# yewzijian/RegTR

Hardware: NVIDIA H100
Metric: pairs/sec on 3DMatch-size clouds (~20k pts); pose err vs ref (higher is better)
Workload: dtype f32

## Files before the change

### include/regtr_b200.h

```cpp
#ifndef REGTR_B200_H_
#define REGTR_B200_H_

#include <stddef.h>
#include <stdint.h>

#ifdef __cplusplus
extern "C" {
#endif

#define REGTR_OK 0
#define REGTR_ERR_ARG (-1)
#define REGTR_ERR_WORKSPACE (-2)
#define REGTR_ERR_UNSUPPORTED (-3)

#define REGTR_STATUS_KEY_RANGE 1u
#define REGTR_STATUS_CAPACITY 2u
#define REGTR_STATUS_GRID 4u
#define REGTR_STATUS_RANGE 8u

int regtr_version(void);
const char* regtr_build_info(void);


size_t regtr_grid_subsample_ws_bytes(int n_cap, int n_clouds);
// ... 11 lines not shown
size_t regtr_cellgrid_state_bytes(int n_cap);
int regtr_cellgrid_build(const float* xyz, const int32_t* offs, int n_clouds, int n_cap, float cell,
                         void* grid, int32_t* order, uint32_t* status,
                         void* ws, size_t ws_bytes, void* state, size_t state_bytes, void* stream);

int regtr_ball_query(const float* q, const int32_t* q_offs, const int32_t* q_order,
                     const float* s, const int32_t* s_offs, const void* s_grid,
                     int n_clouds, int nq_cap, int s_cap, int K, float radius,
                     int32_t* out_idx32, int64_t* out_idx64, void* stream);


size_t regtr_kpconv_ws_bytes(int Nq, int Ns, int Cin);
size_t regtr_kpconv_fwd_ws_bytes(int Nq, int Ns, int Cin, int Cout);
int regtr_kpconv_fwd(const float* q, const float* s, const int32_t* idx, const float* x,
                     const float* W, const float* kp, int Nq, int Ns, const int32_t* nq_dev,
                     const int32_t* ns_dev, int K, int Cin, int Cout,
                     float extent, float* out, void* ws, size_t ws_bytes, void* stream);

int regtr_kpconv_aggregate(const float* q, const float* s, const int32_t* idx, const float* x,
                           const float* kp, int Nq, int Ns, const int32_t* nq_dev, const int32_t* ns_dev,
                           int K, int Cin, float extent,
                           float* wf, uint8_t* rowflag_ws, int flags_ready, void* stream);

int regtr_max_pool(const float* x, const int32_t* idx, int Nq, int Ns, const int32_t* ns_dev, int K, int C,
                   float* out, void* stream);

size_t regtr_instnorm_ws_bytes(int n_cap, int n_clouds, int C);
size_t regtr_instnorm_counter_bytes(int n_clouds, int C);
int regtr_instnorm_act(const float* x, const int32_t* offs, int n_clouds, int n_cap, int C, float eps,
                       const float* res, float slope, float* out, uint8_t* rowflag_out,
                       void* ws, size_t ws_bytes, int32_t* counters, void* stream);

int regtr_instnorm_apply(const float* x, const int32_t* offs, int n_clouds, int n_cap, int C, const float* stats,
                         const float* res, float slope, float* out, uint8_t* rowflag_out, void* stream);


int regtr_split_tf32(const float* x, long long n, float* hi, float* lo, void* stream);

size_t regtr_gemm_ws_bytes(int M, int N, int K);
int regtr_gemm_tf32x3(const float* A, int lda, const float* B_hi, const float* B_lo, int ldb,
                      float* C, int ldc, const float* bias, const float* R, int ldr,
                      int M, int N, int K, const int32_t* m_dev, int relu,
                      void* ws, size_t ws_bytes, void* stream);

size_t regtr_instnorm_part_bytes(int M, int N);
int regtr_gemm_tf32x3_instats(const float* A, int lda, const float* B_hi, const float* B_lo, int ldb,
                              float* C, int ldc, int M, int N, int K, const int32_t* m_dev,
                              const int32_t* offs, int n_clouds, float eps, void* part, float* stats,
                              void* ws, size_t ws_bytes, void* stream);


int regtr_pos_embed_sine(const float* xyz, int n, const float* dim_t, int n_freq, int d_model,
                         float scale, float* out, void* stream);

typedef struct regtr_dropout_args {
    unsigned long long seed, step;
    int32_t pair_base;
    int32_t layer;
    int32_t site;
    uint32_t threshold;
    float scale;
    int32_t n_pairs;
} regtr_dropout_args;

int regtr_layernorm_pos(const float* x, const float* z, const float* gamma, const float* beta, const float* pos, int n,
                        const int32_t* n_dev, const int32_t* offs, int E, float eps, float* y, float* y_pos,
                        float* x_out, const regtr_dropout_args* drop, void* stream);
// ... 354 lines not shown
```

### regtr_b200/csrc/common.cuh

```cuda
#pragma once
#include <cuda_runtime.h>
#include <stdint.h>

#include "../../include/regtr_b200.h"

#define REGTR_NUM_SMS 132

#define REGTR_CHECK_LAUNCH()                                         \
    do {                                                             \
        cudaError_t e__ = cudaGetLastError();                        \
        if (e__ != cudaSuccess) return -(1000 + (int)e__);           \
    } while (0)

static inline int regtr_cdiv(long long a, long long b) { return (int)((a + b - 1) / b); }
static inline size_t regtr_align(size_t x, size_t a = 256) { return (x + a - 1) / a * a; }

__device__ __forceinline__ unsigned long long regtr_pack_key(int cloud, int x, int y, int z) {
    return ((unsigned long long)(unsigned)cloud << 48) | ((unsigned long long)(unsigned)(x + 32768) << 32) |
           ((unsigned long long)(unsigned)(y + 32768) << 16) | (unsigned long long)(unsigned)(z + 32768);
}

__device__ __forceinline__ int regtr_cell_of(float p, float cell) { return (int)floorf(__fdiv_rn(p, cell)); }

__device__ __forceinline__ int regtr_cloud_of(const int32_t* __restrict__ offs, int n_clouds, int i) {
    int lo = 0, hi = n_clouds;
    while (hi - lo > 1) {
        int mid = (lo + hi) >> 1;
        if (offs[mid] <= i) lo = mid; else hi = mid;
    }
    return lo;
}

__device__ __forceinline__ void regtr_row_col(unsigned t, unsigned w, int& row, int& col) {
    if ((w & (w - 1u)) == 0u) { const int sh = 31 - __clz((int)w); row = (int)(t >> sh); col = (int)(t & (w - 1u)); }
    else { row = (int)(t / w); col = (int)(t - (unsigned)row * w); }
}

__device__ __forceinline__ float regtr_tf32_rne(float x) {
    uint32_t u = __float_as_uint(x);
    u += 0x0FFFu + ((u >> 13) & 1u);
    return __uint_as_float(u & 0xFFFFE000u);
}

__device__ __forceinline__ float warp_sum(float v) {
#pragma unroll
    for (int o = 16; o > 0; o >>= 1) v += __shfl_xor_sync(0xffffffffu, v, o);
    return v;
}
__device__ __forceinline__ double warp_sum(double v) {
#pragma unroll
    for (int o = 16; o > 0; o >>= 1) v += __shfl_xor_sync(0xffffffffu, v, o);
    return v;
}
__device__ __forceinline__ float warp_max(float v) {
#pragma unroll
    for (int o = 16; o > 0; o >>= 1) v = fmaxf(v, __shfl_xor_sync(0xffffffffu, v, o));
    return v;
}
```

### regtr_b200/csrc/norm.cu

```cuda
#include "common.cuh"
#include "philox.cuh"

namespace {

constexpr int IN_CH = 128;
constexpr int IN_TY = 8;
constexpr int IN_CT = 128;

__device__ __forceinline__ bool chunk_of(const int32_t* __restrict__ offs, int n_clouds, int chunk, int& cloud,
                                         int& r0, int& r1, int& first, int& count) {
    int acc = 0;
    for (int c = 0; c < n_clouds; ++c) {
        const int a = offs[c], b = offs[c + 1];
        const int nc = (b - a + IN_CH - 1) / IN_CH;
        if (chunk < acc + nc) {
            cloud = c;
            r0 = a + (chunk - acc) * IN_CH;
            r1 = min(r0 + IN_CH, b);
            first = acc;
            count = nc;
            return true;
        }
        acc += nc;
    }
// ... 74 lines not shown
        }
    }
}

__global__ void __launch_bounds__(32 * IN_TY)
k_in_finalize(const int32_t* __restrict__ offs, int n_clouds, int C, float eps, const double2* __restrict__ partial,
              float2* __restrict__ stats) {
    __shared__ double2 red[IN_TY][32];
    const int cloud = blockIdx.x;
    const int c = blockIdx.y * 32 + threadIdx.x;
    int first = 0;
    for (int k = 0; k < cloud; ++k) first += (offs[k + 1] - offs[k] + IN_CH - 1) / IN_CH;
    const int n = offs[cloud + 1] - offs[cloud];
    const int nc = (n + IN_CH - 1) / IN_CH;
    double s = 0.0, ss = 0.0;
    if (c < C) {
        for (int t = threadIdx.y; t < nc; t += IN_TY) {
            const double2 p = partial[(size_t)(first + t) * C + c];
            s += p.x; ss += p.y;
        }
    }
    red[threadIdx.y][threadIdx.x] = make_double2(s, ss);
    __syncthreads();
    if (threadIdx.y == 0 && c < C) {
        for (int t = 1; t < IN_TY; ++t) { s += red[t][threadIdx.x].x; ss += red[t][threadIdx.x].y; }
        const double dn = n > 0 ? (double)n : 1.0;
        const double mean = s / dn;
        double var = ss / dn - mean * mean;
        var = var > 0.0 ? var : 0.0;
        stats[(size_t)cloud * C + c] = make_float2((float)mean, (float)(1.0 / sqrt(var + (double)eps)));
    }
}

template <bool FLAGS>
__global__ void k_in_apply(const float* x, const int32_t* __restrict__ offs, int n_clouds, int n_cap, int C,
                           const float2* __restrict__ stats, const float* res, float slope, float* out,
                           uint8_t* __restrict__ flags) {
    const int c4n = C >> 2;
    const int n_real = offs[n_clouds];
    const unsigned total = (unsigned)min(n_cap, (n_real + 127) & ~127) * (unsigned)c4n;
    const unsigned stride = gridDim.x * blockDim.x;
    for (unsigned t0 = blockIdx.x * blockDim.x; t0 < total; t0 += stride) {
        const unsigned t = t0 + threadIdx.x;
        const bool in_range = t < total;
        int r = 0, c = 0;
        if (in_range) { regtr_row_col(t, (unsigned)c4n, r, c); c *= 4; }
        const size_t o = (size_t)r * C + c;
        const bool live = in_range && r < n_real;
        float y[4] = {0.f, 0.f, 0.f, 0.f};
        if (live) {
            const float4 v = *reinterpret_cast<const float4*>(x + o);
            float4 rv = make_float4(0.f, 0.f, 0.f, 0.f);
            if (res) rv = *reinterpret_cast<const float4*>(res + o);
            const int cloud = regtr_cloud_of(offs, n_clouds, r);
            const float4 st01 = *reinterpret_cast<const float4*>(stats + (size_t)cloud * C + c);
            const float4 st23 = *reinterpret_cast<const float4*>(stats + (size_t)cloud * C + c + 2);
            y[0] = (v.x - st01.x) * st01.y + rv.x; y[1] = (v.y - st01.z) * st01.w + rv.y;
            y[2] = (v.z - st23.x) * st23.y + rv.z; y[3] = (v.w - st23.z) * st23.w + rv.w;
            if (slope >= 0.f) {
#pragma unroll
                for (int j = 0; j < 4; ++j) y[j] = y[j] > 0.f ? y[j] : y[j] * slope;
            }
        }
        if (in_range) *reinterpret_cast<float4*>(out + o) = make_float4(y[0], y[1], y[2], y[3]);
        if (FLAGS) {
            double acc = ((double)y[0] + (double)y[1]) + ((double)y[2] + (double)y[3]);
            for (int d = 1; d < c4n; d <<= 1) acc += __shfl_xor_sync(0xffffffffu, acc, d);
            if (in_range && (threadIdx.x & (c4n - 1)) == 0) flags[r] = live && acc > 0.0;
        }
    }
}

template <int PER, bool DROP = false>
__global__ void k_layernorm_pos(const float* __restrict__ x, const float* __restrict__ gamma,
                                const float* __restrict__ beta, const float* __restrict__ pos, int n,
                                const int32_t* __restrict__ n_dev, int E, float eps, float* __restrict__ y,
                                float* __restrict__ y_pos, const float* __restrict__ z = nullptr,
                                float* __restrict__ x_out = nullptr, DropKey drop = DropKey{}) {
    const int row = (blockIdx.x * blockDim.x + threadIdx.x) >> 5, lane = threadIdx.x & 31;
    if (!DROP && n_dev) n = min(n, *n_dev);
    if (row >= n) return;
    const float* xr = x + (size_t)row * E;
    const int per = E / 32;
    float v[PER], gm[PER], bt[PER], ps[PER];
#pragma unroll
    for (int j = 0; j < PER; ++j)
        if (j < per) {
            const int c = j * 32 + lane;
            v[j] = xr[c]; gm[j] = __ldg(gamma + c); bt[j] = __ldg(beta + c);
            ps[j] = (y_pos && pos) ? pos[(size_t)row * E + c] : 0.f;
        }
    if constexpr (DROP) {
        const int cl = regtr_cloud_of(n_dev, 2 * drop.n_pairs, row);
        const unsigned w1 = drop_word1(drop, cl, 0), rr = (unsigned)(row - n_dev[cl]);
#pragma unroll
// ... 38 lines not shown
    out[t] = o;
}

static inline int in_apply_grid(long long items) {
    const long long b = (items + 255) / 256;
    return (int)(b < 8 * REGTR_NUM_SMS ? (b > 0 ? b : 1) : 8 * REGTR_NUM_SMS);
}

}

extern "C" {

static inline int in_chunks(int n_cap, int n_clouds) { return regtr_cdiv(n_cap > 0 ? n_cap : 1, IN_CH) + n_clouds; }

size_t regtr_instnorm_ws_bytes(int n_cap, int n_clouds, int C) {
    const size_t c = (size_t)(C > 0 ? C : 1), nc = (size_t)(n_clouds > 0 ? n_clouds : 1);
    return regtr_align((size_t)in_chunks(n_cap, (int)nc) * c * sizeof(double2)) + regtr_align(nc * c * sizeof(float2));
}

size_t regtr_instnorm_counter_bytes(int n_clouds, int C) {
    return sizeof(int32_t) * (size_t)(n_clouds > 0 ? n_clouds : 1) * (size_t)regtr_cdiv(C > 0 ? C : 1, IN_CT);
}

int regtr_instnorm_act(const float* x, const int32_t* offs, int n_clouds, int n_cap, int C, float eps,
                       const float* res, float slope, float* out, uint8_t* rowflag_out, void* ws, size_t ws_bytes,
                       int32_t* counters, void* stream_) {
    cudaStream_t st = (cudaStream_t)stream_;
    if (!offs || n_clouds <= 0 || n_cap < 0 || C <= 0) return REGTR_ERR_ARG;
    if (C % 4 != 0 || (long long)n_cap * (C / 4) >= (1ll << 31)) return REGTR_ERR_UNSUPPORTED;
    if (n_cap == 0) return REGTR_OK;
    if (!x || !out || !ws) return REGTR_ERR_ARG;
    if (ws_bytes < regtr_instnorm_ws_bytes(n_cap, n_clouds, C)) return REGTR_ERR_WORKSPACE;
    const int chunks = in_chunks(n_cap, n_clouds);
    double2* partial = (double2*)ws;
    float2* stats = (float2*)((char*)ws + regtr_align((size_t)chunks * C * sizeof(double2)));
    dim3 block(32, IN_TY);
    k_in_stats<<<dim3(chunks, regtr_cdiv(C, IN_CT)), block, 0, st>>>(x, offs, n_clouds, C, partial, counters, eps, stats);
    REGTR_CHECK_LAUNCH();
    if (!counters) {
        k_in_finalize<<<dim3(n_clouds, regtr_cdiv(C, 32)), block, 0, st>>>(offs, n_clouds, C, eps, partial, stats);
        REGTR_CHECK_LAUNCH();
    }
    if (rowflag_out) {
        const int c4n = C / 4;
        if (c4n > 32 || (c4n & (c4n - 1))) return REGTR_ERR_UNSUPPORTED;
        k_in_apply<true><<<in_apply_grid((long long)n_cap * c4n), 256, 0, st>>>(x, offs, n_clouds, n_cap, C, stats,
                                                                                  res, slope, out, rowflag_out);
    } else {
        k_in_apply<false><<<in_apply_grid((long long)n_cap * (C / 4)), 256, 0, st>>>(x, offs, n_clouds, n_cap, C,
                                                                                      stats, res, slope, out, nullptr);
    }
    REGTR_CHECK_LAUNCH();
    return REGTR_OK;
}

int regtr_instnorm_apply(const float* x, const int32_t* offs, int n_clouds, int n_cap, int C, const float* stats,
                         const float* res, float slope, float* out, uint8_t* rowflag_out, void* stream_) {
    cudaStream_t st = (cudaStream_t)stream_;
    if (!offs || n_clouds <= 0 || n_cap < 0 || C <= 0) return REGTR_ERR_ARG;
    if (C % 4 != 0 || (long long)n_cap * (C / 4) >= (1ll << 31)) return REGTR_ERR_UNSUPPORTED;
    if (n_cap == 0) return REGTR_OK;
    if (!x || !out || !stats) return REGTR_ERR_ARG;
    const float2* stp = reinterpret_cast<const float2*>(stats);
    if (rowflag_out) {
        const int c4n = C / 4;
        if (c4n > 32 || (c4n & (c4n - 1))) return REGTR_ERR_UNSUPPORTED;
        k_in_apply<true><<<in_apply_grid((long long)n_cap * c4n), 256, 0, st>>>(x, offs, n_clouds, n_cap, C, stp, res, slope,
                                                                                  out, rowflag_out);
    } else {
        k_in_apply<false><<<in_apply_grid((long long)n_cap * (C / 4)), 256, 0, st>>>(x, offs, n_clouds, n_cap, C, stp, res,
                                                                                      slope, out, nullptr);
    }
    REGTR_CHECK_LAUNCH();
    return REGTR_OK;
}

int regtr_layernorm_pos(const float* x, const float* z, const float* gamma, const float* beta, const float* pos, int n,
                        const int32_t* n_dev, const int32_t* offs, int E, float eps, float* y, float* y_pos,
                        float* x_out, const regtr_dropout_args* drop, void* stream_) {
    cudaStream_t st = (cudaStream_t)stream_;
    if (!z != !drop || !offs != !drop || !x_out != !drop || (drop && n_dev)) return REGTR_ERR_ARG;
    DropKey dk;
    if (drop && (drop_key_of(drop, dk) != REGTR_OK || x_out == x || x_out == z)) return REGTR_ERR_ARG;
    if (n < 0 || E <= 0 || E % 32 != 0 || E > 1024) return REGTR_ERR_ARG;
    if (n == 0) return REGTR_OK;
    if (!x || !gamma || !beta || (!y && !y_pos)) return REGTR_ERR_ARG;
    if (drop && E <= 256)
        k_layernorm_pos<8, true><<<regtr_cdiv((long long)n * 32, 256), 256, 0, st>>>(x, gamma, beta, pos, n, offs, E, eps,
                                                                                     y, y_pos, z, x_out, dk);
    else if (drop)
        k_layernorm_pos<32, true><<<regtr_cdiv((long long)n * 32, 256), 256, 0, st>>>(x, gamma, beta, pos, n, offs, E,
                                                                                      eps, y, y_pos, z, x_out, dk);
    else if (E <= 256)
        k_layernorm_pos<8><<<regtr_cdiv((long long)n * 32, 256), 256, 0, st>>>(x, gamma, beta, pos, n, n_dev, E, eps, y, y_pos);
    else
        k_layernorm_pos<32><<<regtr_cdiv((long long)n * 32, 256), 256, 0, st>>>(x, gamma, beta, pos, n, n_dev, E, eps, y, y_pos);
    REGTR_CHECK_LAUNCH();
    return REGTR_OK;
}

int regtr_pos_embed_sine(const float* xyz, int n, const float* dim_t, int n_freq, int d_model, float scale,
                         float* out, void* stream_) {
    cudaStream_t st = (cudaStream_t)stream_;
// ... 11 lines not shown
```

### regtr_b200/kpconv.py

```python
from __future__ import annotations

import logging
from typing import List

import torch
import torch.nn as nn
import torch.nn.functional as F

from . import ops
from .config import pyramid_plan
from .lazy import LazyDict
from .weights import kernel_disposition

_CELL_SLACK = 1.0001



def level_capacities(cfg, cap0: int, ratio: float = 0.40, quantum: int = 256):
    levels, _, _ = pyramid_plan(cfg)
    caps = [int(cap0)]
    for _ in levels[1:]:
        c = int(caps[-1] * ratio) + 1
        caps.append(min(caps[-1], (c + quantum - 1) // quantum * quantum))
    return caps
# ... 268 lines not shown
        extent = radius * config.KP_extent / config.conv_radius
        self.KPConv = KPConv(config.num_kernel_points, config.in_points_dim, in_dim, out_dim // 2, extent, radius,
                             fixed_kernel_points=config.fixed_kernel_points, KP_influence=config.KP_influence,
                             aggregation_mode=config.aggregation_mode, deformable='deform' in block_name,
                             modulated=config.modulated)
        self.batch_norm = BatchNormBlock(out_dim // 2, config.use_batch_norm, config.batch_norm_momentum)

    def forward(self, x, batch):
        q, s, idx, _, offs_post, nq_dev, ns_dev, nc = _block_io(self, batch)
        y = self.KPConv(q, s, idx, x, nq_dev, ns_dev)
        return self.batch_norm.fuse(y, offs_post, nc, slope=0.1)


class ResnetBottleneckBlock(nn.Module):

    def __init__(self, block_name, in_dim, out_dim, radius, layer_ind, config):
        super().__init__()
        self.block_name, self.layer_ind = block_name, layer_ind
        self.in_dim, self.out_dim = in_dim, out_dim
        bn, mom = config.use_batch_norm, config.batch_norm_momentum
        self.use_bn = bn
        extent = radius * config.KP_extent / config.conv_radius
        mid = out_dim // 4
        self.unary1 = UnaryBlock(in_dim, mid, bn, mom) if in_dim != mid else nn.Identity()
        self.KPConv = KPConv(config.num_kernel_points, config.in_points_dim, mid, mid, extent, radius,
                             fixed_kernel_points=config.fixed_kernel_points, KP_influence=config.KP_influence,
                             aggregation_mode=config.aggregation_mode, deformable='deform' in block_name,
                             modulated=config.modulated)
        self.batch_norm_conv = BatchNormBlock(mid, bn, mom)
        self.unary2 = UnaryBlock(mid, out_dim, bn, mom, no_relu=True)
        self.unary_shortcut = UnaryBlock(in_dim, out_dim, bn, mom, no_relu=True) if in_dim != out_dim \
            else nn.Identity()

    def forward(self, features, batch):
        q, s, idx, offs_pre, offs_post, nq_dev, ns_dev, nc = _block_io(self, batch)
        flags = None
        if isinstance(self.unary1, UnaryBlock) and self.use_bn:
            x, flags, features = self.unary1.fuse(features, offs_pre, nc, m_dev=ns_dev, want_flags=True, skip=True)
        else:
            x = self.unary1.fuse(features, offs_pre, nc, m_dev=ns_dev) if isinstance(self.unary1, UnaryBlock) \
                else features
        if self.use_bn and self.KPConv.out_channels % 32 == 0:
            x, stats = self.KPConv(q, s, idx, x, nq_dev, ns_dev, row_flags=flags, instats=(offs_post, nc))
            x = self.batch_norm_conv.apply(x, stats, offs_post, nc, slope=0.1)
        else:
            x = self.KPConv(q, s, idx, x, nq_dev, ns_dev, row_flags=flags)
            x = self.batch_norm_conv.fuse(x, offs_post, nc, slope=0.1)
        shortcut = ops.max_pool(features, idx, ns_dev) if 'strided' in self.block_name else features
        if isinstance(self.unary_shortcut, UnaryBlock):
            shortcut = self.unary_shortcut.fuse(shortcut, offs_post, nc, m_dev=nq_dev)
        return self.unary2.fuse(x, offs_post, nc, res=shortcut, final_slope=0.1, m_dev=nq_dev)


def block_decider(block_name, radius, in_dim, out_dim, layer_ind, config):
    if block_name in ('simple', 'simple_strided'):
        return SimpleBlock(block_name, in_dim, out_dim, radius, layer_ind, config)
    if block_name in ('resnetb', 'resnetb_strided'):
        return ResnetBottleneckBlock(block_name, in_dim, out_dim, radius, layer_ind, config)
    raise NotImplementedError(f'block {block_name!r} is outside the RegTR hot path (SURVEY.md 2 row 3)')


class KPFEncoder(nn.Module):

    def __init__(self, config, d_bottle, increase_channel_when_downsample=True):
        super().__init__()
        self.logger = logging.getLogger(__name__)
        octave = 0
        r = config.first_subsampling_dl * config.conv_radius
        in_dim, out_dim = config.in_feats_dim, config.first_feats_dim
        self.encoder_blocks = nn.ModuleList()
        self.encoder_skip_dims, self.encoder_skips = [], []
        block = None
        for block_i, block in enumerate(config.architecture):
            if any(t in block for t in ('pool', 'strided', 'upsample', 'global')):
                self.encoder_skips.append(block_i)
                self.encoder_skip_dims.append(in_dim)
            if 'upsample' in block:
                break
            self.encoder_blocks.append(block_decider(block, r, in_dim, out_dim, octave, config))
            in_dim = out_dim // 2 if 'simple' in block else out_dim
            if 'pool' in block or 'strided' in block:
                octave += 1
                r *= 2
                if increase_channel_when_downsample:
                    out_dim *= 2
        if 'upsample' not in block:
            self.encoder_skips.append(block_i)
            self.encoder_skip_dims.append(in_dim)

    def forward(self, x, batch):
        skip_x = []
        for block_i, block_op in enumerate(self.encoder_blocks):
            if block_i in self.encoder_skips:
                skip_x.append(x)
            x = block_op(x, batch)
        return x, skip_x
```

### regtr_b200/lib.py

```python
from __future__ import annotations

import ctypes
import os
import re

import torch

HERE = os.path.dirname(os.path.abspath(__file__))
LIB_PATH = os.path.join(HERE, 'libregtr_b200.so')
HEADER = os.path.join(os.path.dirname(HERE), 'include', 'regtr_b200.h')


class RegtrLibError(RuntimeError):
    pass


_c = ctypes
_P = _c.c_void_p
_I = _c.c_int
_F = _c.c_float
_Z = _c.c_size_t

SIGNATURES = {
    'regtr_version': (_I, []),
    'regtr_build_info': (_c.c_char_p, []),
    'regtr_grid_subsample_ws_bytes': (_Z, [_I, _I]),
    'regtr_grid_subsample_state_bytes': (_Z, [_I]),
    'regtr_grid_subsample': (_I, [_P, _P, _I, _I, _F, _P, _I, _P, _P, _P, _Z, _P, _Z, _P]),
    'regtr_grid_subsample_sorted_ws_bytes': (_Z, [_I]),
    'regtr_grid_subsample_sorted': (_I, [_P, _P, _I, _I, _F, _P, _I, _P, _P, _P, _Z, _P]),
    'regtr_cellgrid_bytes': (_Z, [_I]),
    'regtr_cellgrid_ws_bytes': (_Z, [_I]),
    'regtr_cellgrid_state_bytes': (_Z, [_I]),
    'regtr_cellgrid_build': (_I, [_P, _P, _I, _I, _F, _P, _P, _P, _P, _Z, _P, _Z, _P]),
    'regtr_ball_query': (_I, [_P, _P, _P, _P, _P, _P, _I, _I, _I, _I, _F, _P, _P, _P]),
    'regtr_kpconv_ws_bytes': (_Z, [_I, _I, _I]),
    'regtr_kpconv_fwd_ws_bytes': (_Z, [_I, _I, _I, _I]),
    'regtr_kpconv_fwd': (_I, [_P, _P, _P, _P, _P, _P, _I, _I, _P, _P, _I, _I, _I, _F, _P, _P, _Z, _P]),
    'regtr_kpconv_aggregate': (_I, [_P, _P, _P, _P, _P, _I, _I, _P, _P, _I, _I, _F, _P, _P, _I, _P]),
    'regtr_max_pool': (_I, [_P, _P, _I, _I, _P, _I, _I, _P, _P]),
    'regtr_instnorm_ws_bytes': (_Z, [_I, _I, _I]),
    'regtr_instnorm_counter_bytes': (_Z, [_I, _I]),
    'regtr_instnorm_act': (_I, [_P, _P, _I, _I, _I, _F, _P, _F, _P, _P, _P, _Z, _P, _P]),
    'regtr_instnorm_apply': (_I, [_P, _P, _I, _I, _I, _P, _P, _F, _P, _P, _P]),
    'regtr_instnorm_part_bytes': (_Z, [_I, _I]),
    'regtr_gemm_tf32x3_instats': (_I, [_P, _I, _P, _P, _I, _P, _I, _I, _I, _I, _P, _P, _I, _F, _P, _P, _P, _Z, _P]),
    'regtr_split_tf32': (_I, [_P, _c.c_longlong, _P, _P, _P]),
    'regtr_gemm_ws_bytes': (_Z, [_I, _I, _I]),
    'regtr_gemm_tf32x3': (_I, [_P, _I, _P, _P, _I, _P, _I, _P, _P, _I, _I, _I, _I, _P, _I, _P, _Z, _P]),
    'regtr_pos_embed_sine': (_I, [_P, _I, _P, _I, _I, _F, _P, _P]),
    'regtr_layernorm_pos': (_I, [_P, _P, _P, _P, _P, _I, _P, _P, _I, _F, _P, _P, _P, _P, _P]),
    'regtr_attention_plan': (_I, [_P, _I, _P, _P]),
    'regtr_corr_decode_fwd': (_I, [_P, _P, _I, _P, _P, _P, _P, _P, _P, _I, _I, _I, _I, _I, _F, _P]),
    'regtr_mha_varlen_fwd': (_I, [_P, _I, _P, _I, _P, _I, _P, _I, _P, _P, _P, _P, _P, _I, _I, _P, _I, _I, _I, _F,
                                  _P, _P]),
    'regtr_gemm_tf32x3_qkv_bf16': (_I, [_P, _I, _P, _P, _I, _P, _I, _I, _I, _I, _P, _I, _P, _I, _P, _P]),
    'regtr_mha_bf16_tc_fwd': (_I, [_P, _I, _P, _I, _I, _P, _I, _P, _P, _P, _P, _I, _I, _I, _I, _F, _P]),
    'regtr_gemm_tf32x3_qkv_split': (_I, [_P, _I, _P, _P, _I, _P, _I, _I, _I, _I, _F, _P, _I, _P, _I, _P, _P]),
    'regtr_mha_tf32_tc_fwd': (_I, [_P, _I, _P, _I, _I, _P, _I, _P, _P, _P, _P, _I, _I, _P, _I, _I, _I, _P]),
    'regtr_mha_probs_avg': (_I, [_P, _I, _P, _I, _P, _P, _P, _P, _P, _P, _P, _I, _I, _I, _I, _F, _P]),
    'regtr_mha_varlen_bwd_ws_bytes': (_Z, [_I, _I]),
    'regtr_mha_varlen_bwd': (_I, [_P, _I, _P, _I, _P, _I, _P, _I, _P, _I, _P, _P, _I, _P, _I, _P, _I,
                                  _P, _P, _P, _P, _I, _I, _I, _I, _I, _I, _F, _P, _P, _Z, _P]),
    'regtr_layernorm_bwd_ws_bytes': (_Z, [_I, _I]),
    'regtr_layernorm_bwd': (_I, [_P, _P, _P, _P, _P, _I, _P, _I, _F, _P, _P, _P, _P, _P, _P, _Z, _P]),
    'regtr_relu_bwd': (_I, [_P, _P, _c.c_longlong, _F, _P, _P]),
    'regtr_linear_wgrad_ws_bytes': (_Z, [_I, _I, _I]),
    'regtr_linear_wgrad': (_I, [_P, _I, _P, _I, _I, _I, _I, _P, _P, _P, _Z, _P]),
    'regtr_neighbor_csr_ws_bytes': (_Z, [_I]),
    'regtr_neighbor_csr': (_I, [_P, _I, _I, _I, _P, _P, _P, _Z, _P]),
    'regtr_kpconv_bwd_input_ws_bytes': (_Z, [_I, _I, _I]),
    'regtr_kpconv_bwd_input': (_I, [_P, _P, _P, _P, _P, _P, _I, _I, _I, _I, _F, _P, _P, _P, _P, _P, _Z, _P]),
    'regtr_max_pool_bwd_ws_bytes': (_Z, [_I, _I]),
    'regtr_max_pool_bwd': (_I, [_P, _P, _I, _I, _I, _I, _P, _P, _P, _P, _P, _Z, _P]),
    'regtr_instnorm_bwd_ws_bytes': (_Z, [_I, _I, _I]),
    'regtr_instnorm_bwd': (_I, [_P, _P, _P, _P, _I, _I, _I, _F, _F, _P, _P, _P, _Z, _P]),
    'regtr_grad_norm_ws_bytes': (_Z, [_I]),
# ... 97 lines not shown
```

### regtr_b200/ops.py

```python
from __future__ import annotations

import contextlib
import ctypes
import itertools
import math

import numpy as np
import torch

from . import lib as _lib

_ws_cache = {}

LAUNCHES = 0
KPCONV_TRACE = None
TRACE = None


def _count(n):
    global LAUNCHES
    LAUNCHES += n


def _stream():
# ... 229 lines not shown


def instnorm_act(x, offs, n_clouds: int, res=None, slope: float = -1.0, eps: float = 1e-5, out=None,
                 want_flags: bool = False):
    if _wants_grad(x, res):
        if out is not None:
            raise ValueError('instnorm_act: no out= on the differentiable path')
        y, flags = _InstNormFn.apply(x, res, None, offs, n_clouds, float(slope), float(eps), bool(want_flags))
        return (y, flags) if want_flags else y
    return _instnorm_act_fwd(x, offs, n_clouds, res, slope, eps, out, want_flags)


def _instnorm_act_fwd(x, offs, n_clouds: int, res=None, slope: float = -1.0, eps: float = 1e-5, out=None,
                      want_flags: bool = False):
    L = _lib.load()
    _chk(x, torch.float32, 'x', 2); _chk(offs, torch.int32, 'offs', 1)
    n, C = x.shape
    if res is not None:
        _chk(res, torch.float32, 'res', 2)
    out = torch.empty_like(x) if out is None else out
    nb = L.regtr_instnorm_ws_bytes(n, n_clouds, C)
    ws = workspace(nb, x.device, 'instnorm')
    flags = None
    if want_flags and C // 4 <= 32 and (C // 4) & (C // 4 - 1) == 0:
        flags = torch.empty(max(n, 1), dtype=torch.uint8, device=x.device)
    cnt = workspace(L.regtr_instnorm_counter_bytes(n_clouds, C), x.device, 'instnorm_cnt', zero=True)
    _lib.check(L.regtr_instnorm_act(_p(x), _p(offs), n_clouds, n, C, float(eps), _p(res), float(slope), _p(out),
                                    _p(flags), _p(ws), ws.numel(), _p(cnt), _stream()), 'regtr_instnorm_act')
    _count(2)
    return (out, flags) if want_flags else out


def instnorm_apply(x, offs, n_clouds: int, stats, res=None, slope: float = -1.0, out=None, want_flags: bool = False,
                   eps: float = 1e-5):
    if _wants_grad(x, res):
        if out is not None:
            raise ValueError('instnorm_apply: no out= on the differentiable path')
        y, flags = _InstNormFn.apply(x, res, stats, offs, n_clouds, float(slope), float(eps), bool(want_flags))
        return (y, flags) if want_flags else y
    return _instnorm_apply_fwd(x, offs, n_clouds, stats, res, slope, out, want_flags)


def _instnorm_apply_fwd(x, offs, n_clouds: int, stats, res=None, slope: float = -1.0, out=None,
                        want_flags: bool = False):
    L = _lib.load()
    _chk(x, torch.float32, 'x', 2); _chk(offs, torch.int32, 'offs', 1); _chk(stats, torch.float32, 'stats', 3)
    n, C = x.shape
    out = torch.empty_like(x) if out is None else out
    flags = None
    if want_flags and C // 4 <= 32 and (C // 4) & (C // 4 - 1) == 0:
        flags = torch.empty(max(n, 1), dtype=torch.uint8, device=x.device)
    _lib.check(L.regtr_instnorm_apply(_p(x), _p(offs), n_clouds, n, C, _p(stats), _p(res), float(slope), _p(out),
                                      _p(flags), _stream()), 'regtr_instnorm_apply')
    _count(1)
    return (out, flags) if want_flags else out



def split_weight(w: torch.Tensor, transpose: bool = False):
    L = _lib.load()
    owner = w._base if w._base is not None else w
    cache = owner.__dict__.setdefault('_regtr_split', {})
    key = (w.storage_offset(), tuple(w.shape), tuple(w.stride()), transpose, owner._version)
    hit = cache.get(key)
    if hit is not None:
        return hit
    src = (w.detach().t() if transpose else w.detach()).contiguous().to(torch.float32)
    hi, lo = torch.empty_like(src), torch.empty_like(src)
    _lib.check(L.regtr_split_tf32(_p(src), src.numel(), _p(hi), _p(lo), _stream()), 'regtr_split_tf32')
    _count(1)
    for k in [k for k in cache if k[-1] != owner._version]:
        del cache[k]
    cache[key] = (hi, lo)
    return hi, lo


def gemm(a, b_hi, b_lo, bias=None, residual=None, relu=False, m_dev=None, out=None):
    L = _lib.load()
    if not a.is_cuda or a.dtype != torch.float32 or a.dim() != 2 or a.stride(1) != 1:
        raise ValueError('gemm: A must be a CUDA fp32 matrix with unit column stride')
    M, K = a.shape
    N = b_hi.shape[0]
    out = torch.empty((M, N), dtype=torch.float32, device=a.device) if out is None else out
    nb = L.regtr_gemm_ws_bytes(M, N, K)
    ws = workspace(nb, a.device, 'gemm')
    if TRACE is not None:
# ... 1370 lines not shown
```

### regtr_b200/regtr.py

```python
from __future__ import annotations

import contextlib
import logging
import time
import weakref

import torch
import torch.nn as nn
import torch.nn.functional as F

from . import ops
from .kpconv import KPFEncoder, PreprocessorGPU
from .lazy import LazyDict
from .transformer import (AttentionPlan, PositionEmbeddingCoordsSine, PositionEmbeddingLearned, warn_dropout_eval_only,
                          TransformerCrossEncoder, TransformerCrossEncoderLayer)


class _LossParam(nn.Module):

    def __init__(self, d_embed):
        super().__init__()
        self.W = nn.Parameter(torch.zeros(d_embed, d_embed), requires_grad=True)


# ... 52 lines not shown
        super().__init__()
        self.cfg = cfg
        self.logger = logging.getLogger(self.__class__.__name__)
        self.preprocessor = PreprocessorGPU(cfg)
        self.kpf_encoder = KPFEncoder(cfg, cfg.d_embed)
        self.feat_proj = nn.Linear(self.kpf_encoder.encoder_skip_dims[-1], cfg.d_embed, bias=True)
        if cfg.get('pos_emb_type', 'sine') == 'sine':
            self.pos_embed = PositionEmbeddingCoordsSine(3, cfg.d_embed, scale=cfg.get('pos_emb_scaling', 1.0))
        elif cfg['pos_emb_type'] == 'learned':
            self.pos_embed = PositionEmbeddingLearned(3, cfg.d_embed)
        else:
            raise NotImplementedError
        layer = TransformerCrossEncoderLayer(
            cfg.d_embed, cfg.nhead, cfg.d_feedforward, cfg.dropout, activation=cfg.transformer_act,
            normalize_before=cfg.pre_norm, sa_val_has_pos_emb=cfg.sa_val_has_pos_emb,
            ca_val_has_pos_emb=cfg.ca_val_has_pos_emb, attention_type=cfg.attention_type,
            attention_impl=cfg.get('attention_impl', 'fp32'))
        norm = nn.LayerNorm(cfg.d_embed) if cfg.pre_norm else None
        self.transformer_encoder = TransformerCrossEncoder(layer, cfg.num_encoder_layers, norm,
                                                           return_intermediate=True)
        if cfg.get('direct_regress_coor', False):
            self.correspondence_decoder = CorrespondenceRegressor(cfg.d_embed)
        else:
            self.correspondence_decoder = CorrespondenceDecoder(cfg.d_embed, cfg.corr_decoder_has_pos_emb,
                                                                self.pos_embed)
        if cfg.feature_loss_type == 'infonce':
            self.feature_criterion = _LossParam(cfg.d_embed)
            self.feature_criterion_un = _LossParam(cfg.d_embed)

    @property
    def device(self):
        return next(self.parameters()).device

    def _stage_encoder(self, meta):
        pts = meta['_points']
        feats0 = torch.ones_like(pts[0][:, 0:1])
        feats_un, _ = self.kpf_encoder(feats0, meta)
        nd = meta.get('_ndev')
        both_un = ops.linear(feats_un, self.feat_proj.weight, self.feat_proj.bias,
                             m_dev=nd[-1] if nd else None)
        xyz_c = pts[-1]
        pe = self.pos_embed(xyz_c)
        return dict(both_un=both_un.contiguous(), xyz_c=xyz_c, pe=pe)

    def _stage_attention(self, enc, plan: AttentionPlan):
        cfg = self.cfg
        cond = self.transformer_encoder.forward_packed(
            enc['both_un'], enc['pe'] if cfg.transformer_encoder_has_pos_emb else None, plan)
        corr, logit = self.correspondence_decoder.forward_packed(cond, enc['xyz_c'], enc['pe'], plan)
        return dict(cond=cond, corr=corr, logit=logit)

    def _stage_pose(self, enc, att, offs_c, B: int):
        return ops.pose_from_corr(enc['xyz_c'], att['corr'].contiguous(), att['logit'][..., 0].contiguous(), offs_c, B)

    def _core(self, meta, B: int, plan: AttentionPlan):
        enc = self._stage_encoder(meta)
        att = self._stage_attention(enc, plan)
        pose = self._stage_pose(enc, att, meta['_offs'][-1], B)
        return dict(both_un=enc['both_un'], xyz_c=enc['xyz_c'], cond=att['cond'], corr=att['corr'],
                    logit=att['logit'], pose=pose)

    @staticmethod
    def _assemble(core, lens_c, B):
        n = sum(lens_c)
        split = lambda t, dim=0: torch.split(t.narrow(dim, 0, n), lens_c, dim=dim)
        un, kp = split(core['both_un']), split(core['xyz_c'])
        feat, warped, ovl = split(core['cond'], 1), split(core['corr'], 1), split(core['logit'], 1)
        out = PackedOutput({
            'src_feat_un': un[:B], 'tgt_feat_un': un[B:],
            'src_feat': list(feat[:B]), 'tgt_feat': list(feat[B:]),
# ... 54 lines not shown
            unsupported.append('direct_regress_coor=False (CorrespondenceDecoder)')
        if cfg.get('pos_emb_type', 'sine') != 'sine':
            unsupported.append(f"pos_emb_type={cfg['pos_emb_type']!r}")
        if not (cfg.sa_val_has_pos_emb and cfg.ca_val_has_pos_emb):
            unsupported.append('sa/ca_val_has_pos_emb=False')
        if cfg.get('attention_impl', 'fp32') != 'fp32':
            unsupported.append(f"attention_impl={cfg['attention_impl']!r}")
        if unsupported:
            raise NotImplementedError('forward_train: no backward for ' + ', '.join(unsupported))

    def _stage_attention_train(self, feats_un, xyz_c, offs_c, B: int, plan: AttentionPlan, drop=None):
        cfg = self.cfg
        both_un = ops.linear(feats_un, self.feat_proj.weight, self.feat_proj.bias)
        with torch.no_grad():
            pe = self.pos_embed(xyz_c)
        cond = self.transformer_encoder.forward_train_packed(
            both_un, pe if cfg.transformer_encoder_has_pos_emb else None, plan, drop=drop)
        corr, logit = self.correspondence_decoder.forward_packed(cond, xyz_c, pe, plan)
        with torch.no_grad():
            pose = ops.pose_from_corr(xyz_c, corr.detach().contiguous(), logit.detach()[..., 0].contiguous(), offs_c, B)
        return dict(both_un=both_un, xyz_c=xyz_c, cond=cond, corr=corr, logit=logit, pose=pose)

    def forward_train(self, batch, train_encoder: bool = False, *, dropout_key=None):
        if self.transformer_encoder.record_attentions:
            raise RuntimeError('forward_train: attention maps are recorded by the eager inference forward only; set '
                               'transformer_encoder.record_attentions = False to train')
        self._check_trainable(train_encoder)
        B = len(batch['src_xyz'])
        with torch.no_grad():
            meta = self.preprocessor(list(batch['src_xyz']) + list(batch['tgt_xyz']), lazy_upsamples=True)
            batch['kpconv_meta'] = meta
        pts = meta['_points']
        with contextlib.nullcontext() if train_encoder else torch.no_grad():
            feats_un, _ = self.kpf_encoder(torch.ones_like(pts[0][:, 0:1]), meta)
        lens_c = meta['_lens'][-1]
        plan = AttentionPlan(lens_c, pts[-1].device)
        drop = None
        p = self.transformer_encoder.dropout_p
        if self.training and p > 0.0:
            if dropout_key is None:
                dropout_key = (int(torch.randint(0, 2 ** 62, (1,)).item()), 0, 0)
            seed, step, pair_base = dropout_key
            drop = ops.DropoutKey(p, seed, step, pair_base, B, offs=meta['_offs'][-1], max_len=plan.max_len)
        core = self._stage_attention_train(feats_un, pts[-1], meta['_offs'][-1], B, plan, drop)
        return self._assemble(core, lens_c, B)

    @torch.no_grad()
    def forward(self, batch):
        warn_dropout_eval_only(self)
        B = len(batch['src_xyz'])
        meta = self.preprocessor(list(batch['src_xyz']) + list(batch['tgt_xyz']), lazy_upsamples=True)
        batch['kpconv_meta'] = meta
        lens_c = meta['_lens'][-1]
        plan = AttentionPlan(lens_c, meta['_points'][-1].device)
        return self._assemble(self._core(meta, B, plan), lens_c, B)


class GraphedRegTR:

    STAGES = ('preprocess', 'encoder', 'attention_decoder', 'pose')

    def __init__(self, model: RegTR, bucket: int = 8192, full_meta: bool = True, ratio: float = 0.30,
                 retry_ratio: float = 0.45, stages: bool = False):
        self.model = model
        self.bucket = int(bucket)
        self.full_meta = full_meta
        self.ratio, self.retry_ratio = ratio, retry_ratio
# ... 23 lines not shown
            ops.release_namespace(st['ns'])
        graphs.clear()

    def _drop(self, key):
        st = self.graphs.pop(key, None)
        if st is not None:
            torch.cuda.synchronize(self.model.device)
            ops.release_namespace(st['ns'])

    def _capture(self, B: int, cap0: int):
        ns = ops.new_namespace()
        with ops.scratch_namespace(ns):
            st = self._capture_impl(B, cap0)
        st['ns'] = ns
        return st

    def _capture_impl(self, B: int, cap0: int):
        from .kpconv import level_capacities
        model = self.model
        dev = model.device
        caps = level_capacities(model.cfg, cap0, ratio=self.ratios.get((B, cap0), self.ratio))
        st = dict(points=torch.zeros((cap0, 3), dtype=torch.float32, device=dev),
                  offs0=torch.zeros(2 * B + 1, dtype=torch.int32, device=dev), caps=caps)
        box = {}

        def s_pre():
            box['pyr'] = model.preprocessor.build(st['points'], st['offs0'], 2 * B, caps=caps,
                                                  want64=self.full_meta, upsamples=False,
                                                  dense=(B, cap0) not in self.sparse)
            box['plan'] = AttentionPlan.from_device(box['pyr'].offs_all[-1], B, caps[-1])
            box['meta'] = box['pyr'].private(static=True)

        def s_enc():
            box['enc'] = model._stage_encoder(box['meta'])

        def s_att():
            box['att'] = model._stage_attention(box['enc'], box['plan'])

        def s_pose():
            pyr = box['pyr']
            box['pose'] = model._stage_pose(box['enc'], box['att'], box['meta']['_offs'][-1], B)
            box['tail'] = torch.cat([pyr.offs_all.reshape(-1), pyr.status.view(torch.int32),
                                     box['pose'].reshape(-1).view(torch.int32)])

        fns = [s_pre, s_enc, s_att, s_pose]

        def run():
            for f in fns:
                f()

        side = torch.cuda.Stream(device=dev)
        side.wait_stream(torch.cuda.current_stream(dev))
        with torch.cuda.stream(side):
            n = cap0 // (2 * B)
            st['offs0'].copy_(torch.arange(0, 2 * B + 1, dtype=torch.int32, device=dev) * n)
            st['points'].uniform_(-1.0, 1.0)
            for _ in range(2):
                run()
        torch.cuda.current_stream(dev).wait_stream(side)
        torch.cuda.synchronize(dev)
        n0 = ops.LAUNCHES
        graphs = []
        if self.stages:
            pool = None
            for f in fns:
                g = torch.cuda.CUDAGraph()
                with torch.cuda.graph(g, pool=pool):
# ... 154 lines not shown
```

Baseline: 861.0.

## Fold shortcut max-pool and instance norm into the residual apply kernel

Adds a folded inference path for KPConv bottleneck blocks. The shortcut's instance-norm and the strided max-pool are now computed when the final instnorm-apply kernel reads its residual, and the unary2 output uses the GEMM-with-stats path. This removes separate normalise and pool passes and the intermediate shortcut tensors they write. In exchange the apply kernel does a K-wide gathered max per element and reads extra stats. The arithmetic is reordered into fma form, which can change rounding slightly.

Result: no change. 870.1, median of 6 (+1.1%).

```diff
diff --git a/include/regtr_b200.h b/include/regtr_b200.h
--- a/include/regtr_b200.h
+++ b/include/regtr_b200.h
@@ -67,7 +67,8 @@
                        void* ws, size_t ws_bytes, int32_t* counters, void* stream);
 
 int regtr_instnorm_apply(const float* x, const int32_t* offs, int n_clouds, int n_cap, int C, const float* stats,
-                         const float* res, float slope, float* out, uint8_t* rowflag_out, void* stream);
+                         const float* res, const float* res_stats, const int32_t* res_idx, int res_K, int res_Ns,
+                         const int32_t* res_ns_dev, float slope, float* out, uint8_t* rowflag_out, void* stream);
 
 
 int regtr_split_tf32(const float* x, long long n, float* hi, float* lo, void* stream);
diff --git a/regtr_b200/csrc/common.cuh b/regtr_b200/csrc/common.cuh
--- a/regtr_b200/csrc/common.cuh
+++ b/regtr_b200/csrc/common.cuh
@@ -42,6 +42,14 @@
     return __uint_as_float(u & 0xFFFFE000u);
 }
 
+__device__ __forceinline__ float regtr_in_norm(float v, float m, float r, float res) {
+    return __fmaf_rn(__fsub_rn(v, m), r, res);
+}
+
+__device__ __forceinline__ float regtr_leaky(float y, float slope) {
+    return slope >= 0.f ? (y > 0.f ? y : __fmul_rn(y, slope)) : y;
+}
+
 __device__ __forceinline__ float warp_sum(float v) {
 #pragma unroll
     for (int o = 16; o > 0; o >>= 1) v += __shfl_xor_sync(0xffffffffu, v, o);
diff --git a/regtr_b200/csrc/norm.cu b/regtr_b200/csrc/norm.cu
--- a/regtr_b200/csrc/norm.cu
+++ b/regtr_b200/csrc/norm.cu
@@ -130,12 +130,21 @@
     }
 }
 
+struct InRes {
+    const float* x;
+    const float2* stats;
+    const int32_t* idx;
+    int K, Ns;
+    const int32_t* ns_dev;
+};
+
 template <bool FLAGS>
 __global__ void k_in_apply(const float* x, const int32_t* __restrict__ offs, int n_clouds, int n_cap, int C,
-                           const float2* __restrict__ stats, const float* res, float slope, float* out,
+                           const float2* __restrict__ stats, InRes res, float slope, float* out,
                            uint8_t* __restrict__ flags) {
     const int c4n = C >> 2;
     const int n_real = offs[n_clouds];
+    const int res_ns = res.ns_dev ? min(res.Ns, *res.ns_dev) : res.Ns;
     const unsigned total = (unsigned)min(n_cap, (n_real + 127) & ~127) * (unsigned)c4n;
     const unsigned stride = gridDim.x * blockDim.x;
     for (unsigned t0 = blockIdx.x * blockDim.x; t0 < total; t0 += stride) {
@@ -148,17 +157,31 @@
         float y[4] = {0.f, 0.f, 0.f, 0.f};
         if (live) {
             const float4 v = *reinterpret_cast<const float4*>(x + o);
+            const int cloud = regtr_cloud_of(offs, n_clouds, r);
             float4 rv = make_float4(0.f, 0.f, 0.f, 0.f);
-            if (res) rv = *reinterpret_cast<const float4*>(res + o);
-            const int cloud = regtr_cloud_of(offs, n_clouds, r);
+            if (res.idx) {
+                rv = make_float4(-INFINITY, -INFINITY, -INFINITY, -INFINITY);
+                for (int k = 0; k < res.K; ++k) {
+                    const int id = res.idx[(size_t)r * res.K + k];
+                    float4 p = make_float4(0.f, 0.f, 0.f, 0.f);
+                    if (id >= 0 && id < res_ns) p = __ldg(reinterpret_cast<const float4*>(res.x + (size_t)id * C + c));
+                    rv.x = fmaxf(rv.x, p.x); rv.y = fmaxf(rv.y, p.y); rv.z = fmaxf(rv.z, p.z); rv.w = fmaxf(rv.w, p.w);
+                }
+            } else if (res.x) {
+                rv = *reinterpret_cast<const float4*>(res.x + o);
+                if (res.stats) {
+                    const float4 r01 = *reinterpret_cast<const float4*>(res.stats + (size_t)cloud * C + c);
+                    const float4 r23 = *reinterpret_cast<const float4*>(res.stats + (size_t)cloud * C + c + 2);
+                    rv.x = regtr_in_norm(rv.x, r01.x, r01.y, 0.f); rv.y = regtr_in_norm(rv.y, r01.z, r01.w, 0.f);
+                    rv.z = regtr_in_norm(rv.z, r23.x, r23.y, 0.f); rv.w = regtr_in_norm(rv.w, r23.z, r23.w, 0.f);
+                }
+            }
             const float4 st01 = *reinterpret_cast<const float4*>(stats + (size_t)cloud * C + c);
             const float4 st23 = *reinterpret_cast<const float4*>(stats + (size_t)cloud * C + c + 2);
-            y[0] = (v.x - st01.x) * st01.y + rv.x; y[1] = (v.y - st01.z) * st01.w + rv.y;
-            y[2] = (v.z - st23.x) * st23.y + rv.z; y[3] = (v.w - st23.z) * st23.w + rv.w;
-            if (slope >= 0.f) {
-#pragma unroll
-                for (int j = 0; j < 4; ++j) y[j] = y[j] > 0.f ? y[j] : y[j] * slope;
-            }
+            y[0] = regtr_leaky(regtr_in_norm(v.x, st01.x, st01.y, rv.x), slope);
+            y[1] = regtr_leaky(regtr_in_norm(v.y, st01.z, st01.w, rv.y), slope);
+            y[2] = regtr_leaky(regtr_in_norm(v.z, st23.x, st23.y, rv.z), slope);
+            y[3] = regtr_leaky(regtr_in_norm(v.w, st23.z, st23.w, rv.w), slope);
         }
         if (in_range) *reinterpret_cast<float4*>(out + o) = make_float4(y[0], y[1], y[2], y[3]);
         if (FLAGS) {
@@ -263,6 +286,7 @@
     if (!x || !out || !ws) return REGTR_ERR_ARG;
     if (ws_bytes < regtr_instnorm_ws_bytes(n_cap, n_clouds, C)) return REGTR_ERR_WORKSPACE;
     const int chunks = in_chunks(n_cap, n_clouds);
+    const InRes rs = {res, nullptr, nullptr, 0, 0, nullptr};
     double2* partial = (double2*)ws;
     float2* stats = (float2*)((char*)ws + regtr_align((size_t)chunks * C * sizeof(double2)));
     dim3 block(32, IN_TY);
@@ -276,30 +300,37 @@
         const int c4n = C / 4;
         if (c4n > 32 || (c4n & (c4n - 1))) return REGTR_ERR_UNSUPPORTED;
         k_in_apply<true><<<in_apply_grid((long long)n_cap * c4n), 256, 0, st>>>(x, offs, n_clouds, n_cap, C, stats,
-                                                                                  res, slope, out, rowflag_out);
+                                                                                  rs, slope, out, rowflag_out);
     } else {
         k_in_apply<false><<<in_apply_grid((long long)n_cap * (C / 4)), 256, 0, st>>>(x, offs, n_clouds, n_cap, C,
-                                                                                      stats, res, slope, out, nullptr);
+                                                                                      stats, rs, slope, out, nullptr);
     }
     REGTR_CHECK_LAUNCH();
     return REGTR_OK;
 }
 
 int regtr_instnorm_apply(const float* x, const int32_t* offs, int n_clouds, int n_cap, int C, const float* stats,
-                         const float* res, float slope, float* out, uint8_t* rowflag_out, void* stream_) {
+                         const float* res, const float* res_stats, const int32_t* res_idx, int res_K, int res_Ns,
+                         const int32_t* res_ns_dev, float slope, float* out, uint8_t* rowflag_out, void* stream_) {
     cudaStream_t st = (cudaStream_t)stream_;
     if (!offs || n_clouds <= 0 || n_cap < 0 || C <= 0) return REGTR_ERR_ARG;
+    if ((res_stats || res_idx) && !res) return REGTR_ERR_ARG;
+    if (res_stats && res_idx) return REGTR_ERR_ARG;
+    if (res_idx && (res_K <= 0 || res_Ns < 0)) return REGTR_ERR_ARG;
     if (C % 4 != 0 || (long long)n_cap * (C / 4) >= (1ll << 31)) return REGTR_ERR_UNSUPPORTED;
     if (n_cap == 0) return REGTR_OK;
     if (!x || !out || !stats) return REGTR_ERR_ARG;
+    if (res_idx && (res == out || res == x)) return REGTR_ERR_ARG;
     const float2* stp = reinterpret_cast<const float2*>(stats);
+    const InRes rs = {res, reinterpret_cast<const float2*>(res_stats), res_idx, res_idx ? res_K : 0, res_Ns,
+                      res_idx ? res_ns_dev : nullptr};
     if (rowflag_out) {
         const int c4n = C / 4;
         if (c4n > 32 || (c4n & (c4n - 1))) return REGTR_ERR_UNSUPPORTED;
-        k_in_apply<true><<<in_apply_grid((long long)n_cap * c4n), 256, 0, st>>>(x, offs, n_clouds, n_cap, C, stp, res, slope,
+        k_in_apply<true><<<in_apply_grid((long long)n_cap * c4n), 256, 0, st>>>(x, offs, n_clouds, n_cap, C, stp, rs, slope,
                                                                                   out, rowflag_out);
     } else {
-        k_in_apply<false><<<in_apply_grid((long long)n_cap * (C / 4)), 256, 0, st>>>(x, offs, n_clouds, n_cap, C, stp, res,
+        k_in_apply<false><<<in_apply_grid((long long)n_cap * (C / 4)), 256, 0, st>>>(x, offs, n_clouds, n_cap, C, stp, rs,
                                                                                       slope, out, nullptr);
     }
     REGTR_CHECK_LAUNCH();
diff --git a/regtr_b200/kpconv.py b/regtr_b200/kpconv.py
--- a/regtr_b200/kpconv.py
+++ b/regtr_b200/kpconv.py
@@ -324,7 +324,7 @@
         self.unary_shortcut = UnaryBlock(in_dim, out_dim, bn, mom, no_relu=True) if in_dim != out_dim \
             else nn.Identity()
 
-    def forward(self, features, batch):
+    def forward(self, features, batch, fold_norm=False):
         q, s, idx, offs_pre, offs_post, nq_dev, ns_dev, nc = _block_io(self, batch)
         flags = None
         if isinstance(self.unary1, UnaryBlock) and self.use_bn:
@@ -338,10 +338,25 @@
         else:
             x = self.KPConv(q, s, idx, x, nq_dev, ns_dev, row_flags=flags)
             x = self.batch_norm_conv.fuse(x, offs_post, nc, slope=0.1)
+        if fold_norm and self.use_bn and self.out_dim % 32 == 0 and not torch.is_grad_enabled():
+            return self._unary2_folded(x, features, idx, offs_post, nq_dev, ns_dev, nc)
         shortcut = ops.max_pool(features, idx, ns_dev) if 'strided' in self.block_name else features
         if isinstance(self.unary_shortcut, UnaryBlock):
             shortcut = self.unary_shortcut.fuse(shortcut, offs_post, nc, m_dev=nq_dev)
         return self.unary2.fuse(x, offs_post, nc, res=shortcut, final_slope=0.1, m_dev=nq_dev)
+
+    def _unary2_folded(self, x, features, idx, offs_post, nq_dev, ns_dev, nc):
+        shortcut, res_kw = features, {}
+        if 'strided' in self.block_name:
+            if isinstance(self.unary_shortcut, UnaryBlock):
+                shortcut = ops.max_pool(features, idx, ns_dev)
+            else:
+                res_kw = dict(res_pool=(idx, ns_dev))
+        if isinstance(self.unary_shortcut, UnaryBlock):
+            shortcut, sc_stats = ops.linear_instats(shortcut, self.unary_shortcut.mlp.weight, offs_post, nc, m_dev=nq_dev)
+            res_kw = dict(res_stats=sc_stats)
+        y, stats = ops.linear_instats(x, self.unary2.mlp.weight, offs_post, nc, m_dev=nq_dev)
+        return ops.instnorm_apply(y, offs_post, nc, stats, res=shortcut, slope=0.1, **res_kw)
 
 
 def block_decider(block_name, radius, in_dim, out_dim, layer_ind, config):
@@ -380,10 +395,11 @@
             self.encoder_skips.append(block_i)
             self.encoder_skip_dims.append(in_dim)
 
-    def forward(self, x, batch):
+    def forward(self, x, batch, fold_norm=False):
         skip_x = []
         for block_i, block_op in enumerate(self.encoder_blocks):
             if block_i in self.encoder_skips:
                 skip_x.append(x)
-            x = block_op(x, batch)
+            x = block_op(x, batch, fold_norm=True) if fold_norm and isinstance(block_op, ResnetBottleneckBlock) \
+                else block_op(x, batch)
         return x, skip_x
diff --git a/regtr_b200/lib.py b/regtr_b200/lib.py
--- a/regtr_b200/lib.py
+++ b/regtr_b200/lib.py
@@ -42,7 +42,7 @@
     'regtr_instnorm_ws_bytes': (_Z, [_I, _I, _I]),
     'regtr_instnorm_counter_bytes': (_Z, [_I, _I]),
     'regtr_instnorm_act': (_I, [_P, _P, _I, _I, _I, _F, _P, _F, _P, _P, _P, _Z, _P, _P]),
-    'regtr_instnorm_apply': (_I, [_P, _P, _I, _I, _I, _P, _P, _F, _P, _P, _P]),
+    'regtr_instnorm_apply': (_I, [_P, _P, _I, _I, _I, _P, _P, _P, _P, _I, _I, _P, _F, _P, _P, _P]),
     'regtr_instnorm_part_bytes': (_Z, [_I, _I]),
     'regtr_gemm_tf32x3_instats': (_I, [_P, _I, _P, _P, _I, _P, _I, _I, _I, _I, _P, _P, _I, _F, _P, _P, _P, _Z, _P]),
     'regtr_split_tf32': (_I, [_P, _c.c_longlong, _P, _P, _P]),
diff --git a/regtr_b200/ops.py b/regtr_b200/ops.py
--- a/regtr_b200/ops.py
+++ b/regtr_b200/ops.py
@@ -285,26 +285,36 @@
 
 
 def instnorm_apply(x, offs, n_clouds: int, stats, res=None, slope: float = -1.0, out=None, want_flags: bool = False,
-                   eps: float = 1e-5):
+                   eps: float = 1e-5, res_stats=None, res_pool=None):
     if _wants_grad(x, res):
-        if out is not None:
-            raise ValueError('instnorm_apply: no out= on the differentiable path')
+        if out is not None or res_stats is not None or res_pool is not None:
+            raise ValueError('instnorm_apply: no out= and no residual computed on read on the differentiable path')
         y, flags = _InstNormFn.apply(x, res, stats, offs, n_clouds, float(slope), float(eps), bool(want_flags))
         return (y, flags) if want_flags else y
-    return _instnorm_apply_fwd(x, offs, n_clouds, stats, res, slope, out, want_flags)
+    return _instnorm_apply_fwd(x, offs, n_clouds, stats, res, slope, out, want_flags, res_stats, res_pool)
 
 
 def _instnorm_apply_fwd(x, offs, n_clouds: int, stats, res=None, slope: float = -1.0, out=None,
-                        want_flags: bool = False):
+                        want_flags: bool = False, res_stats=None, res_pool=None):
     L = _lib.load()
     _chk(x, torch.float32, 'x', 2); _chk(offs, torch.int32, 'offs', 1); _chk(stats, torch.float32, 'stats', 3)
     n, C = x.shape
+    if (res_stats is not None or res_pool is not None) and res is None:
+        raise ValueError('instnorm_apply: res_stats / res_pool need res')
+    idx, ns_dev = res_pool if res_pool is not None else (None, None)
+    if idx is not None:
+        _chk(res, torch.float32, 'res', 2); _chk(idx, torch.int32, 'res_pool idx', 2)
+        if res.shape[1] != C or idx.shape[0] < n:
+            raise ValueError('instnorm_apply: the pooled residual needs C columns and an index row per output row')
+    if res_stats is not None:
+        _chk(res_stats, torch.float32, 'res_stats', 3)
     out = torch.empty_like(x) if out is None else out
     flags = None
     if want_flags and C // 4 <= 32 and (C // 4) & (C // 4 - 1) == 0:
         flags = torch.empty(max(n, 1), dtype=torch.uint8, device=x.device)
-    _lib.check(L.regtr_instnorm_apply(_p(x), _p(offs), n_clouds, n, C, _p(stats), _p(res), float(slope), _p(out),
-                                      _p(flags), _stream()), 'regtr_instnorm_apply')
+    _lib.check(L.regtr_instnorm_apply(_p(x), _p(offs), n_clouds, n, C, _p(stats), _p(res), _p(res_stats), _p(idx),
+                                      idx.shape[1] if idx is not None else 0, res.shape[0] if idx is not None else 0,
+                                      _p(ns_dev), float(slope), _p(out), _p(flags), _stream()), 'regtr_instnorm_apply')
     _count(1)
     return (out, flags) if want_flags else out
 
diff --git a/regtr_b200/regtr.py b/regtr_b200/regtr.py
--- a/regtr_b200/regtr.py
+++ b/regtr_b200/regtr.py
@@ -108,10 +108,10 @@
     def device(self):
         return next(self.parameters()).device
 
-    def _stage_encoder(self, meta):
+    def _stage_encoder(self, meta, fold_norm=False):
         pts = meta['_points']
         feats0 = torch.ones_like(pts[0][:, 0:1])
-        feats_un, _ = self.kpf_encoder(feats0, meta)
+        feats_un, _ = self.kpf_encoder(feats0, meta, fold_norm=fold_norm)
         nd = meta.get('_ndev')
         both_un = ops.linear(feats_un, self.feat_proj.weight, self.feat_proj.bias,
                              m_dev=nd[-1] if nd else None)
@@ -232,7 +232,8 @@
             batch['kpconv_meta'] = meta
         pts = meta['_points']
         with contextlib.nullcontext() if train_encoder else torch.no_grad():
-            feats_un, _ = self.kpf_encoder(torch.ones_like(pts[0][:, 0:1]), meta)
+            feats_un, _ = self.kpf_encoder(torch.ones_like(pts[0][:, 0:1]), meta,
+                                           fold_norm=not train_encoder)
         lens_c = meta['_lens'][-1]
         plan = AttentionPlan(lens_c, pts[-1].device)
         drop = None
@@ -322,7 +323,7 @@
             box['meta'] = box['pyr'].private(static=True)
 
         def s_enc():
-            box['enc'] = model._stage_encoder(box['meta'])
+            box['enc'] = model._stage_encoder(box['meta'], fold_norm=True)
 
         def s_att():
             box['att'] = model._stage_attention(box['enc'], box['plan'])
```
